# starkware-libs/stark-perpetual

Measured on AMD Instinct MI355X. Metric: pedersen_hashes_per_sec, higher is better.
Workload: dtype u32x9; 1 GPU; 2^16-leaf Pedersen Merkle rebuild per GPU (BASELINE.json configs[1]), 63 rebuilds in lockstep; tree_height=16, leaves_per_gpu=65536, calls_per_region=28, streams=2, window_bits=26, combine=none

## Files before the change

stark-perpetual_amd/csrc/pedersen.hip:

```cpp
#include <algorithm>
#include <cstdlib>
#include <cstring>
#include <map>
#include <vector>

#include "context.hpp"
#include "pedersen.hpp"
#include "quad.hpp"
#include "ragged_plan.hpp"

#ifndef SP_ACC_WAVES
#define SP_ACC_WAVES 1
#endif

namespace sp {

struct raw_aff {
  u256 x, y;
};
__device__ __forceinline__ raw_aff ld_raw(const aff_packed* e) {
  const uint4* q = reinterpret_cast<const uint4*>(e);
  const uint4 a = q[0], b = q[1], c = q[2], d = q[3];
  raw_aff r;
  r.x.w[0] = a.x; r.x.w[1] = a.y; r.x.w[2] = a.z; r.x.w[3] = a.w;
// ... 364 lines not shown
  const int wa = (upper && cnt >= 3) ? q + 2 * QUADS : q;
  const int wb = (upper && cnt >= 4) ? q + 3 * QUADS : q + QUADS;
  const aff pa = entry(wa), pb = entry(wb);
  qpt p = qmmadd(pa.x, pa.y, pb.x, pb.y, k);
  if (upper && cnt == 3) {
    p.a = odd ? pa.y : pa.x;
    p.b = FE_ONE_M;
  }
  qpt s = qadd<false>(p, k);
  if (cnt == 2) {
    s.a = fe_dpp<quad_perm(0, 1, 0, 1)>(p.a);
    s.b = fe_dpp<quad_perm(0, 1, 0, 1)>(p.b);
  }
  for (int j = 4; j < max_cnt; ++j) {
    const aff pj = entry(j < cnt ? q + j * QUADS : q);
    qpt t;
    t.a = fe_sel(upper, odd ? pj.y : pj.x, s.a);
    t.b = fe_sel(upper, FE_ONE_M, s.b);
    const qpt u = qadd<false>(t, k);
    if (j < cnt) s = u;
  }
#define SP_BUTTERFLY(XORV, LAST)                               \
  {                                                            \
    qpt t;                                                     \
    t.a = fe_sel(upper, fe_swizzle_xor<XORV>(s.a), s.a);       \
    t.b = fe_sel(upper, fe_swizzle_xor<XORV>(s.b), s.b);       \
    s = qadd<LAST>(t, k);                                      \
  }
  if constexpr (LOG_Q == 1) SP_BUTTERFLY(4, true)
  if constexpr (LOG_Q == 2) { SP_BUTTERFLY(4, false) SP_BUTTERFLY(8, true) }
  if constexpr (LOG_Q == 3) { SP_BUTTERFLY(4, false) SP_BUTTERFLY(8, false) SP_BUTTERFLY(16, true) }
#undef SP_BUTTERFLY
  const fe zinv = fe_inv_quad<true>(s.b, k);
  *unhashable = limbs_is_zero(zinv);
  return fe_pack(fe_canon(fe_mul(s.a, zinv)));
}

template <int LOG_Q, bool SPARSE = false>
__global__ void __launch_bounds__(256)
ped_quad_kernel(const uint64_t* __restrict__ x, const uint64_t* __restrict__ y, size_t xstride, size_t ystride,
                size_t n, const aff_packed* __restrict__ ped, int w0, int log2e, int nwin_plan,
                uint8_t* __restrict__ status, unsigned* __restrict__ flag, const int2* __restrict__ src,
                uint64_t* __restrict__ out, size_t ostride, int dup, const aff_packed* __restrict__ cpts, int cx,
                int cy) {
  constexpr int QUADS = 1 << LOG_Q, LANES = 4 * QUADS;
  const size_t gt = (size_t)blockIdx.x * blockDim.x + threadIdx.x;
  const size_t e_raw = gt / ((size_t)LANES << dup);
  const int g = (int)(gt % LANES);
  const bool active = e_raw < n;
  const size_t e = active ? e_raw : n - 1;
  const uint64_t *fx, *fy;
  operand_pointers(x, y, xstride, ystride, src, e, fx, fy);
  int mode = 0;
  if constexpr (SPARSE) {
    const int2 sc = src[e];
    mode = sc.x < 0 ? 1 : (sc.y < 0 ? 2 : 0);
  }
  bool unhashable;
  const u256 xa_plain = quad_hash<LOG_Q, SPARSE>(fx, fy, mode, cpts, cx, cy, ped, w0, log2e, nwin_plan, g, &unhashable);
  uint8_t st = unhashable ? SP_HASH_UNHASHABLE : SP_HASH_OK;
  if (!active || g != 0) return;
  if (!u256_lt(ld_u256(fx), U256_P) || !u256_lt(ld_u256(fy), U256_P)) st = SP_HASH_OUT_OF_RANGE;
  st_u256(out + 4 * e * ostride, xa_plain);
  if (status) status[e] = st;
  if (st != SP_HASH_OK && flag) atomicOr(flag, (unsigned)st);
}

template <int LOG_Q, bool SPARSE>
__global__ void __launch_bounds__(256)
ped_path_kernel(uint64_t* __restrict__ felts, const uint64_t* __restrict__ emp, size_t n,
                const aff_packed* __restrict__ ped, int w0, int log2e, int nwin_plan, unsigned* __restrict__ flag,
                const int2* __restrict__ src_all, PathLevels pl, int dup, const aff_packed* __restrict__ cpts_tree,
                int cx, int cy) {
  constexpr int QUADS = 1 << LOG_Q, LANES = 4 * QUADS;
  __shared__ uint64_t slot[256 / LANES][4];
  const size_t gt = (size_t)blockIdx.x * blockDim.x + threadIdx.x;
  const size_t e_raw = gt / ((size_t)LANES << dup);
  const int g = (int)(gt % LANES), grp = (int)(threadIdx.x / LANES);
  const bool active = e_raw < n;
  const size_t e = active ? e_raw : n - 1;
  for (int i = 0; i < pl.n_levels; ++i) {
    const int l = pl.first + i;
    const int2 sc = src_all[pl.src_off[l] + e];
    const uint64_t* y = emp + 4 * l;
    const uint64_t* fx = sc.x >= 0 ? felts + 4 * (size_t)sc.x : y;
    const uint64_t* fy = sc.y >= 0 ? felts + 4 * (size_t)sc.y : y;
    if (i > 0) {
      if (sc.x == pl.val_base[l] + (int)e) fx = slot[grp];
      else fy = slot[grp];
    }
    int mode = 0;
    if constexpr (SPARSE) mode = sc.x < 0 ? 1 : (sc.y < 0 ? 2 : 0);
    bool unhashable;
    const u256 xa = quad_hash<LOG_Q, SPARSE>(fx, fy, mode, cpts_tree ? cpts_tree + 2 * l : nullptr, cx, cy, ped, w0, log2e,
                                             nwin_plan, g, &unhashable);
    uint8_t st = unhashable ? SP_HASH_UNHASHABLE : SP_HASH_OK;
    if (i == 0 && g == 0 && (!u256_lt(ld_u256(fx), U256_P) || !u256_lt(ld_u256(fy), U256_P))) st = SP_HASH_OUT_OF_RANGE;
    __syncthreads();
    if (g == 0) {
      uint32_t* sl = reinterpret_cast<uint32_t*>(slot[grp]);
#pragma unroll
      for (int w = 0; w < 8; ++w) sl[w] = xa.w[w];
      if (active) {
        st_u256(felts + 4 * ((size_t)pl.val_base[l + 1] + e), xa);
        if (st != SP_HASH_OK && flag) atomicOr(flag, (unsigned)st);
      }
    }
    __syncthreads();
  }
}

template <int LOG_Q>
__global__ void __launch_bounds__(256)
ped_chain_kernel(const uint64_t* __restrict__ first, const uint64_t* __restrict__ words, long long word_stride, size_t n,
                 int steps, bool h_right, const aff_packed* __restrict__ ped, int w0, int log2e, int nwin_plan,
                 unsigned* __restrict__ flag, uint64_t* __restrict__ out, int dup) {
  constexpr int QUADS = 1 << LOG_Q, LANES = 4 * QUADS;
  __shared__ uint64_t slot[256 / LANES][4];
  const size_t gt = (size_t)blockIdx.x * blockDim.x + threadIdx.x;
  const size_t e_raw = gt / ((size_t)LANES << dup);
  const int g = (int)(gt % LANES), grp = (int)(threadIdx.x / LANES);
  const bool active = e_raw < n;
  const size_t e = active ? e_raw : n - 1;
  const uint64_t* h = first + 4 * e;
  const uint64_t* w = words + 4 * e;
  for (int j = 0; j < steps; ++j, w += 4 * word_stride) {
    const uint64_t* fx = h_right ? w : h;
    const uint64_t* fy = h_right ? h : w;
    bool unhashable;
    const u256 xa = quad_hash<LOG_Q, false>(fx, fy, 0, nullptr, 0, 0, ped, w0, log2e, nwin_plan, g, &unhashable);
    uint8_t st = unhashable ? SP_HASH_UNHASHABLE : SP_HASH_OK;
    if (g == 0 && (!u256_lt(ld_u256(w), U256_P) || (j == 0 && !u256_lt(ld_u256(h), U256_P)))) st = SP_HASH_OUT_OF_RANGE;
    __syncthreads();
    if (g == 0) {
      uint32_t* sl = reinterpret_cast<uint32_t*>(slot[grp]);
#pragma unroll
      for (int k = 0; k < 8; ++k) sl[k] = xa.w[k];
      if (active) {
        if (j == steps - 1) st_u256(out + 4 * e, xa);
        if (st != SP_HASH_OK && flag) atomicOr(flag, (unsigned)st);
      }
    }
    __syncthreads();
    h = slot[grp];
  }
}

__device__ __forceinline__ bool u256_same(const u256& a, const u256& b) {
  uint32_t d = 0;
#pragma unroll
  for (int k = 0; k < 8; ++k) d |= a.w[k] ^ b.w[k];
  return d == 0;
}
template <bool SIDED>
__device__ __forceinline__ void fold_result(size_t e, const u256& v, uint8_t st, uint64_t* __restrict__ out,
                                            uint8_t* __restrict__ status, const uint64_t* __restrict__ expect,
                                            size_t estride, uint8_t* __restrict__ verdict) {
  st_u256(out + 4 * e, v);
  if (status) status[e] = st;
  if constexpr (SIDED) {
    if (verdict) verdict[e] = (st == SP_HASH_OK && u256_same(v, ld_u256(expect + 4 * e * estride))) ? SP_PATH_TRUE : SP_PATH_FALSE;
  }
}

template <int LOG_Q, bool SIDED>
__global__ void __launch_bounds__(256)
ped_fold_ragged_kernel(const uint64_t* __restrict__ leaves, const uint64_t* __restrict__ words,
                       const uint32_t* __restrict__ off, const uint64_t* __restrict__ keys, size_t n,
                       const aff_packed* __restrict__ ped, int w0, int log2e, int nwin_plan, unsigned* __restrict__ flag,
                       uint8_t* __restrict__ status, uint64_t* __restrict__ out, const uint64_t* __restrict__ expect,
                       size_t estride, uint8_t* __restrict__ verdict, int dup) {
  constexpr int QUADS = 1 << LOG_Q, LANES = 4 * QUADS;
  __shared__ uint64_t slot[256 / LANES][4];
  __shared__ int block_steps;
  const size_t gt = (size_t)blockIdx.x * blockDim.x + threadIdx.x;
  const size_t e_raw = gt / ((size_t)LANES << dup);
  const int g = (int)(gt % LANES), grp = (int)(threadIdx.x / LANES);
  const bool active = e_raw < n;
  const size_t e = active ? e_raw : n - 1;
  const bool writer = active && g == 0 && ((gt / LANES) & (((size_t)1 << dup) - 1)) == 0;
  const uint32_t o0 = off[e];
  const int steps = (int)(off[e + 1] - o0) - (SIDED ? 0 : 1);
  uint64_t key = 0;
  if constexpr (SIDED) key = keys[e];
  if (threadIdx.x == 0) block_steps = 0;
  __syncthreads();
  if (g == 0 && steps > 0) atomicMax(&block_steps, steps);
  __syncthreads();
  const int bound = block_steps;
  const uint64_t* leaf = SIDED ? leaves + 4 * e : words + 4 * (size_t)o0;
  uint8_t st = SP_HASH_OK;
  if (steps == 0 && writer) {
    const u256 v = ld_u256(leaf);
    if (!u256_lt(v, U256_P)) st = SP_HASH_OUT_OF_RANGE;
    fold_result<SIDED>(e, v, st, out, status, expect, estride, verdict);
    if (st != SP_HASH_OK && flag) atomicOr(flag, (unsigned)st);
  }
  const uint64_t* h = leaf;
  const uint64_t* w = SIDED ? words + 4 * (size_t)o0 : leaf + 4;
  for (int j = 0; j < bound; ++j, w += 4) {
    const bool live = j < steps;
    const bool right = SIDED && ((key >> (j & 63)) & 1) != 0;
    const uint64_t* fx = live ? (right ? w : h) : leaf;
    const uint64_t* fy = live ? (right ? h : w) : leaf;
    bool unhashable;
    const u256 xa = quad_hash<LOG_Q, false>(fx, fy, 0, nullptr, 0, 0, ped, w0, log2e, nwin_plan, g, &unhashable);
    if (live && g == 0) {
      if (!u256_lt(ld_u256(w), U256_P) || (j == 0 && !u256_lt(ld_u256(h), U256_P))) st |= SP_HASH_OUT_OF_RANGE;
      else if (unhashable) st |= SP_HASH_UNHASHABLE;
    }
    __syncthreads();
    if (live && g == 0) {
      uint32_t* sl = reinterpret_cast<uint32_t*>(slot[grp]);
#pragma unroll
      for (int k = 0; k < 8; ++k) sl[k] = xa.w[k];
      if (j == steps - 1 && writer) {
        fold_result<SIDED>(e, xa, st, out, status, expect, estride, verdict);
        if (st != SP_HASH_OK && flag) atomicOr(flag, (unsigned)st);
      }
    }
    __syncthreads();
    h = slot[grp];
  }
}

__global__ void __launch_bounds__(256)
ped_fold_ragged_scatter_kernel(const uint64_t* __restrict__ work, const uint64_t* __restrict__ lone, bool sided,
                               const uint32_t* __restrict__ off, const uint32_t* __restrict__ perm,
                               const uint32_t* __restrict__ step_off, const uint8_t* __restrict__ step_status, size_t n,
                               unsigned* __restrict__ flag, uint8_t* __restrict__ status, uint64_t* __restrict__ out,
                               const uint64_t* __restrict__ expect, size_t estride, uint8_t* __restrict__ verdict) {
  const size_t k = (size_t)blockIdx.x * blockDim.x + threadIdx.x;
  if (k >= n) return;
  const uint32_t c = perm[k];
  const uint32_t o0 = off[c], steps = off[c + 1] - o0 - (sided ? 0 : 1);
  uint8_t st = SP_HASH_OK;
  u256 v;
  if (steps == 0) {
    v = ld_u256(lone + 4 * (size_t)(sided ? c : o0));
    if (!u256_lt(v, U256_P)) st = SP_HASH_OUT_OF_RANGE;
    if (st != SP_HASH_OK && flag) atomicOr(flag, (unsigned)st);
  } else {
    v = ld_u256(work + 4 * k);
    for (uint32_t s = 0; s < steps; ++s) st |= step_status[(size_t)step_off[s] + k];
  }
  fold_result<true>(c, v, st, out, status, expect, estride, verdict);
}

__global__ void __launch_bounds__(256)
ped_top_kernel(uint64_t* __restrict__ cur, size_t n_in, int n_levels, const aff_packed* __restrict__ ped, int w0, int log2e,
               int nwin_plan, unsigned* __restrict__ flag) {
  constexpr int LANES = 32, GROUPS = 256 / LANES;
  __shared__ uint64_t slot[2][GROUPS][4];
  const int g = (int)(threadIdx.x % LANES), grp = (int)(threadIdx.x / LANES);
  const size_t b = blockIdx.x;
  const int chunk = 1 << n_levels;
  uint64_t* out = cur + 4 * n_in;
  size_t n_out = n_in >> 1;
  int share = 4 - n_levels;
  for (int t = 0; t < n_levels; ++t, ++share) {
    const int cnt = chunk >> (t + 1);
    const int i = grp >> share;
    const bool writer = g == 0 && (grp & ((1 << share) - 1)) == 0;
    const uint64_t *fx, *fy;
    if (t == 0) {
      fx = cur + 4 * ((size_t)chunk * b + 2 * (size_t)i);
      fy = fx + 4;
    } else {
      fx = slot[(t - 1) & 1][2 * i];
      fy = slot[(t - 1) & 1][2 * i + 1];
    }
    bool unhashable;
    const u256 xa = quad_hash<3, false>(fx, fy, 0, nullptr, 0, 0, ped, w0, log2e, nwin_plan, g, &unhashable);
    uint8_t st = unhashable ? SP_HASH_UNHASHABLE : SP_HASH_OK;
    if (t == 0 && writer && (!u256_lt(ld_u256(fx), U256_P) || !u256_lt(ld_u256(fy), U256_P))) st = SP_HASH_OUT_OF_RANGE;
    if (writer) {
      uint32_t* sl = reinterpret_cast<uint32_t*>(slot[t & 1][i]);
#pragma unroll
      for (int w = 0; w < 8; ++w) sl[w] = xa.w[w];
      st_u256(out + 4 * ((size_t)cnt * b + (size_t)i), xa);
      if (st != SP_HASH_OK && flag) atomicOr(flag, (unsigned)st);
    }
    __syncthreads();
    out += 4 * n_out;
    n_out >>= 1;
  }
}

template <int S>
__device__ __forceinline__ u256 tail_hash(const uint64_t* fx, const uint64_t* fy, int lane, const aff_packed* __restrict__ ped,
                                          int w0, int log2e, int nwin, uint8_t* st) {
  if constexpr (S < 3) {
    return split_fused_x<S>(split_accumulate<S>(fx, fy, lane, ped, w0, log2e, nwin), st);
  } else {
    bool unhashable;
    const u256 xa = quad_hash<S - 2, false>(fx, fy, 0, nullptr, 0, 0, ped, w0, log2e, nwin, lane, &unhashable);
    if (unhashable) *st = SP_HASH_UNHASHABLE;
    return xa;
  }
}

__global__ void __launch_bounds__(256)
ped_tail_kernel(uint64_t* __restrict__ cur, size_t n_in, int s0, int n_levels, const aff_packed* __restrict__ ped, int w0,
                int log2e, int nwin_plan, unsigned* __restrict__ flag) {
  __shared__ uint64_t slot[2][256][4];
  const size_t b = blockIdx.x;
  const int tid = (int)threadIdx.x;
  uint64_t* out = cur + 4 * n_in;
  size_t n_out = n_in >> 1;
#pragma unroll 1
  for (int t = 0; t < n_levels; ++t) {
    const int s = s0 + t;
    const int cls = s < 5 ? s : 5;
    const int cnt = 256 >> s;
    const int i = tid >> s, lane = tid & ((1 << cls) - 1);
    const bool writer = (tid & ((1 << s) - 1)) == 0;
    const uint64_t *fx, *fy;
    if (t == 0) {
      fx = cur + 4 * (2 * (size_t)cnt * b + 2 * (size_t)i);
      fy = fx + 4;
    } else {
      fx = slot[(t - 1) & 1][2 * i];
      fy = slot[(t - 1) & 1][2 * i + 1];
    }
    uint8_t st = SP_HASH_OK;
    u256 xa;
    switch (cls) {
      case 0: xa = tail_hash<0>(fx, fy, lane, ped, w0, log2e, nwin_plan, &st); break;
      case 1: xa = tail_hash<1>(fx, fy, lane, ped, w0, log2e, nwin_plan, &st); break;
      case 2: xa = tail_hash<2>(fx, fy, lane, ped, w0, log2e, nwin_plan, &st); break;
      case 3: xa = tail_hash<3>(fx, fy, lane, ped, w0, log2e, nwin_plan, &st); break;
      case 4: xa = tail_hash<4>(fx, fy, lane, ped, w0, log2e, nwin_plan, &st); break;
      default: xa = tail_hash<5>(fx, fy, lane, ped, w0, log2e, nwin_plan, &st); break;
    }
    if (t == 0 && writer && (!u256_lt(ld_u256(fx), U256_P) || !u256_lt(ld_u256(fy), U256_P))) st = SP_HASH_OUT_OF_RANGE;
    if (writer) {
      uint32_t* sl = reinterpret_cast<uint32_t*>(slot[t & 1][i]);
#pragma unroll
      for (int w = 0; w < 8; ++w) sl[w] = xa.w[w];
      st_u256(out + 4 * ((size_t)cnt * b + (size_t)i), xa);
      if (st != SP_HASH_OK && flag) atomicOr(flag, (unsigned)st);
    }
    __syncthreads();
    out += 4 * n_out;
    n_out >>= 1;
  }
}

__global__ void __launch_bounds__(256)
ped_finish_kernel(const int32_t* __restrict__ sX, int32_t* __restrict__ sZZ, int32_t* __restrict__ sPre,
                  size_t n, size_t T, uint64_t* __restrict__ out, size_t ostride,
                  uint8_t* __restrict__ status, unsigned* __restrict__ flag) {
  const size_t t = (size_t)blockIdx.x * blockDim.x + threadIdx.x;
  if (t >= T) return;
  const size_t cnt = t < n ? (n - t + T - 1) / T : 0;
  fe run = FE_ONE_M;
  if (cnt > 0) {
    fe znext = load_limbs(sZZ, n, t);
#pragma unroll 1
    for (size_t j = 0; j < cnt; ++j) {
      const size_t e = t + j * T;
      const fe z = znext;
      if (j + 1 < cnt) znext = load_limbs(sZZ, n, e + T);
      store_limbs(sPre, n, e, run);
      run = fe_mul(run, z);
    }
  }
  if (fe_is_zero(run)) {
    run = FE_ONE_M;
#pragma unroll 1
    for (size_t e = t; e < n; e += T) {
      fe z = load_limbs(sZZ, n, e);
      if (fe_is_zero(z)) {
        z = FE_ONE_M;
        store_limbs(sZZ, n, e, z);
        if (status) status[e] = SP_HASH_UNHASHABLE;
        if (flag) atomicOr(flag, (unsigned)SP_HASH_UNHASHABLE);
      }
      store_limbs(sPre, n, e, run);
      run = fe_mul(run, z);
    }
  }
  size_t e = cnt > 0 ? t + (cnt - 1) * T : 0;
  fe zn = run, pn = run, xn = run;
  if (cnt > 0) {
    zn = load_limbs(sZZ, n, e);
    pn = load_limbs(sPre, n, e);
    xn = load_limbs(sX, n, e);
  }
  fe inv = fe_inv_shared_quad<2, true>(run, (int)(threadIdx.x & 3));
#pragma unroll 1
  for (size_t j = cnt; j-- > 0;) {
    const fe z = zn, pre = pn, xv = xn;
    const size_t cur = t + j * T;
    if (j > 0) {
      zn = load_limbs(sZZ, n, cur - T);
      pn = load_limbs(sPre, n, cur - T);
      xn = load_limbs(sX, n, cur - T);
    }
    const fe zinv = fe_mul(inv, pre);
    inv = fe_mul(inv, z);
    const fe xa = fe_mul(xv, zinv);
    st_u256(out + 4 * cur * ostride, fe_pack(fe_canon(xa)));
  }
}

template <bool Z_IN_LDS>
__global__ void __launch_bounds__(256)
ped_finish_lds_kernel(const int32_t* __restrict__ sX, int32_t* __restrict__ sZZ, size_t n, size_t T,
                      uint64_t* __restrict__ out, size_t ostride, uint8_t* __restrict__ status,
                      unsigned* __restrict__ flag, int kmax) {
  extern __shared__ int32_t fin_lds[];
  int32_t* lpre = fin_lds;
  int32_t* lz = fin_lds + (size_t)kmax * NL * 256;
  auto lds_put = [&](int32_t* base, size_t j, const fe& v) {
#pragma unroll
    for (int k = 0; k < NL; ++k) base[((j * NL + k) << 8) + threadIdx.x] = v.l[k];
  };
  auto lds_get = [&](const int32_t* base, size_t j) {
    fe v;
#pragma unroll
    for (int k = 0; k < NL; ++k) v.l[k] = base[((j * NL + k) << 8) + threadIdx.x];
    return v;
  };
  const size_t t = (size_t)blockIdx.x * blockDim.x + threadIdx.x;
  if (t >= T) return;
  const size_t cnt = t < n ? (n - t + T - 1) / T : 0;
  fe run = FE_ONE_M;
  if (cnt > 0) {
    fe znext = load_limbs(sZZ, n, t);
#pragma unroll 1
    for (size_t j = 0; j < cnt; ++j) {
      const fe z = znext;
      if (j + 1 < cnt) znext = load_limbs(sZZ, n, t + (j + 1) * T);
      lds_put(lpre, j, run);
      if (Z_IN_LDS) lds_put(lz, j, z);
      run = fe_mul(run, z);
    }
  }
  if (fe_is_zero(run)) {
    run = FE_ONE_M;
    size_t j = 0;
#pragma unroll 1
    for (size_t e = t; e < n; e += T, ++j) {
      fe z = load_limbs(sZZ, n, e);
      if (fe_is_zero(z)) {
        z = FE_ONE_M;
        store_limbs(sZZ, n, e, z);
        if (status) status[e] = SP_HASH_UNHASHABLE;
        if (flag) atomicOr(flag, (unsigned)SP_HASH_UNHASHABLE);
      }
      lds_put(lpre, j, run);
      if (Z_IN_LDS) lds_put(lz, j, z);
      run = fe_mul(run, z);
    }
  }
  size_t e = cnt > 0 ? t + (cnt - 1) * T : 0;
  fe zn = run, xn = run;
  if (cnt > 0) {
    if (!Z_IN_LDS) zn = load_limbs(sZZ, n, e);
    xn = load_limbs(sX, n, e);
  }
  fe inv = fe_inv_shared_quad<2, true>(run, (int)(threadIdx.x & 3));
#pragma unroll 1
  for (size_t j = cnt; j-- > 0;) {
    const fe z = Z_IN_LDS ? lds_get(lz, j) : zn, xv = xn;
    const fe pre = lds_get(lpre, j);
    const size_t cur = t + j * T;
    if (j > 0) {
      if (!Z_IN_LDS) zn = load_limbs(sZZ, n, cur - T);
      xn = load_limbs(sX, n, cur - T);
    }
    const fe zinv = fe_mul(inv, pre);
    inv = fe_mul(inv, z);
    const fe xa = fe_mul(xv, zinv);
    st_u256(out + 4 * cur * ostride, fe_pack(fe_canon(xa)));
  }
}

__global__ void __launch_bounds__(128)
ped_point_kernel(const uint64_t* __restrict__ x, const uint64_t* __restrict__ y, size_t n,
                 const aff_packed* __restrict__ ped, int w0, int log2e, int nwin,
                 uint64_t* __restrict__ ox, uint64_t* __restrict__ oy, uint8_t* __restrict__ status) {
  size_t e = (size_t)blockIdx.x * blockDim.x + threadIdx.x;
  if (e >= n) e = n - 1;
  u256 sx = ld_u256(x + 4 * e);
  u256 sy = ld_u256(y + 4 * e);
  if (!u256_lt(sx, U256_P) || !u256_lt(sy, U256_P)) {
    status[e] = SP_HASH_OUT_OF_RANGE;
    return;
  }
  bits512 str = concat_xy(sx, sy);
  xyzz acc = xyzz_from_aff(ld_aff(ped + pop_bits(str, w0)));
  for (int g = 1; g < nwin; ++g) {
    const window_ref r = window_entry(ped, g, pop_bits(str, log2e + 1), w0, log2e);
    acc = xyzz_madd(acc, signed_aff(ld_raw(r.entry), r.negative));
  }
  if (fe_is_zero(acc.ZZ)) {
    status[e] = SP_HASH_UNHASHABLE;
    return;
  }
  const fe izzz = fe_inv(acc.ZZZ);
  st_u256(ox + 4 * e, fe_pack(fe_from_mont(fe_mul(acc.X, fe_sqr(fe_mul(acc.ZZ, izzz))))));
  st_u256(oy + 4 * e, fe_pack(fe_from_mont(fe_mul(acc.Y, izzz))));
  status[e] = SP_HASH_OK;
}

__global__ void __launch_bounds__(64)
ped_partial_kernel(const uint64_t* __restrict__ felts, int count, const aff_packed* __restrict__ ped, int w0, int log2e,
                   int nwin, int cx, int cy, aff_packed* __restrict__ out) {
  int t = (int)(blockIdx.x * blockDim.x + threadIdx.x);
  if (t >= 2 * count) t = 2 * count - 1;
  const int side = t & 1;
  const uint64_t* f = felts + 4 * (size_t)(t >> 1);
  const int g0 = side == 0 ? 0 : nwin - cy, g1 = side == 0 ? cx : nwin;
  auto entry = [&](int w) {
    const window_ref r =
        window_entry(ped, w, window_from_memory(f, f, window_start(w, w0, log2e), window_width(w, w0, log2e)), w0, log2e);
    return signed_aff(ld_raw(r.entry), r.negative);
  };
  aff_packed res;
  if (g1 - g0 == 1) {
    const aff a = entry(g0);
    res.x = fe_pack(fe_canon(a.x));
    res.y = fe_pack(fe_canon(a.y));
  } else {
    xyzz acc = xyzz_mmadd(entry(g0), entry(g0 + 1));
    for (int g = g0 + 2; g < g1; ++g) acc = xyzz_madd(acc, entry(g));
    const fe izzz = fe_inv(acc.ZZZ);
    const fe izz = fe_sqr(fe_mul(acc.ZZ, izzz));
    res.x = fe_pack(fe_canon(fe_mul(acc.X, izz)));
    res.y = fe_pack(fe_canon(fe_mul(acc.Y, izzz)));
  }
  uint4* q = reinterpret_cast<uint4*>(out + t);
  q[0] = make_uint4(res.x.w[0], res.x.w[1], res.x.w[2], res.x.w[3]);
  q[1] = make_uint4(res.x.w[4], res.x.w[5], res.x.w[6], res.x.w[7]);
  q[2] = make_uint4(res.y.w[0], res.y.w[1], res.y.w[2], res.y.w[3]);
  q[3] = make_uint4(res.y.w[4], res.y.w[5], res.y.w[6], res.y.w[7]);
}

struct KernelProfile {
  bool enabled = false;
  std::vector<hipEvent_t> ev;
  std::vector<size_t> units;
  size_t used = 0;
};
static KernelProfile g_prof;
bool profile_launch_begin(hipStream_t st) {
  if (!g_prof.enabled || g_prof.used + 2 > g_prof.ev.size()) return false;
  (void)hipEventRecord(g_prof.ev[g_prof.used], st);
  return true;
}
void profile_launch_end(hipStream_t st, size_t units) {
  (void)hipEventRecord(g_prof.ev[g_prof.used + 1], st);
  g_prof.units.push_back(units);
  g_prof.used += 2;
}
static bool g_split_enabled = getenv("STARKPERP_NO_SPLIT") == nullptr;
static bool g_fuse_enabled = getenv("STARKPERP_NO_FUSE") == nullptr;
static bool g_quad_enabled = getenv("STARKPERP_NO_QUAD") == nullptr;
static bool g_quad2_enabled = getenv("STARKPERP_NO_QUAD2") == nullptr;
static bool g_level_split = getenv("STARKPERP_NO_LEVEL_SPLIT") == nullptr;
static bool g_quad_no_dup = getenv("STARKPERP_QUAD_NO_DUP") != nullptr;
static bool g_sparse_enabled = getenv("STARKPERP_NO_SPARSE_LEVELS") == nullptr;
static size_t g_quad_max = getenv("STARKPERP_QUAD_MAX") ? (size_t)atoll(getenv("STARKPERP_QUAD_MAX")) : 2048;
static size_t quad_class_max(int log_q, int nwin) {
  if (!g_quad_enabled || nwin > 64) return 0;
  if (log_q == 3) return nwin >= 16 ? g_quad_max : 0;
  if (log_q == 2) return nwin >= 8 ? 2 * g_quad_max : 0;
  return nwin >= 4 && g_quad2_enabled ? 4 * g_quad_max : 0;
}
struct QuadShape {
  int log_q, dup;
  unsigned blocks;
};
static QuadShape quad_shape(size_t n, int nwin) {
  QuadShape q{0, 0, 0};
  for (int l = 3; l >= 1 && q.log_q == 0; --l) {
    if (n <= quad_class_max(l, nwin)) q.log_q = l;
  }
  if (q.log_q == 0) return q;
  while ((4 << (q.log_q + q.dup)) < 64 && ((n * 4) << (q.log_q + q.dup + 1)) <= 65536) ++q.dup;
  if (g_quad_no_dup) q.dup = 0;
  q.blocks = (unsigned)((((n * 4) << (q.log_q + q.dup)) + 255) / 256);
  return q;
}
template <class F>
static void dispatch_quad(int log_q, bool sparse, F&& launch) {
  using std::integral_constant;
  if (sparse && log_q == 2) launch(integral_constant<int, 2>{}, std::true_type{});
  else if (sparse) launch(integral_constant<int, 1>{}, std::true_type{});
  else if (log_q == 3) launch(integral_constant<int, 3>{}, std::false_type{});
  else if (log_q == 2) launch(integral_constant<int, 2>{}, std::false_type{});
  else launch(integral_constant<int, 1>{}, std::false_type{});
}

static std::map<StreamKey, DeviceBuffer> g_stream_scratch;
static int get_scratch(size_t n, Scratch& s, hipStream_t st) { return get_scratch_public(n, s, st); }
static int get_scratch_tail(size_t n, size_t tail_bytes, Scratch& s, char** tail, hipStream_t st) {
  DeviceBuffer& buf = g_stream_scratch[stream_key(st)];
  const size_t plane = ((9 * n * sizeof(int32_t)) + 255) & ~(size_t)255;
  SP_HIP(buf.reserve(3 * plane + 256 + tail_bytes));
  char* b = (char*)buf.ptr;
  s.X = (int32_t*)b;
  s.ZZ = (int32_t*)(b + plane);
  s.Pre = (int32_t*)(b + 2 * plane);
  s.flag = (unsigned*)(b + 3 * plane);
  if (tail) *tail = b + 3 * plane + 256;
  return SP_OK;
}
int get_scratch_public(size_t n, Scratch& s, hipStream_t st) { return get_scratch_tail(n, 0, s, nullptr, st); }

static size_t g_finish_lanes = getenv("STARKPERP_FINISH_LANES") ? (size_t)atoll(getenv("STARKPERP_FINISH_LANES")) : 65536;
static size_t parse_split_lanes() {
  const char* e = getenv("STARKPERP_SPLIT_LANES");
  long long v = e ? atoll(e) : 65536;
  if (v < 256) v = 256;
  if (v > (1ll << 24)) v = 1ll << 24;
  return ((size_t)v + 255) & ~(size_t)255;
}
static size_t g_split_lanes = parse_split_lanes();
static bool g_finish_lds = getenv("STARKPERP_NO_FINISH_LDS") == nullptr;
static int finish_lds_ready() {
  static std::map<int, int> done;
  int dev = -1;
  if (hipGetDevice(&dev) != hipSuccess) return SP_ERR_HIP;
  auto it = done.find(dev);
  if (it != done.end()) return it->second;
  const int want = 16 * NL * 256 * (int)sizeof(int32_t);
  hipError_t e = hipFuncSetAttribute(reinterpret_cast<const void*>(ped_finish_lds_kernel<true>),
                                     hipFuncAttributeMaxDynamicSharedMemorySize, want);
  if (e == hipSuccess)
    e = hipFuncSetAttribute(reinterpret_cast<const void*>(ped_finish_lds_kernel<false>),
                            hipFuncAttributeMaxDynamicSharedMemorySize, want);
  if (e != hipSuccess) (void)hipGetLastError();
  return done[dev] = (e == hipSuccess ? SP_OK : SP_ERR_HIP);
}
static size_t finish_threads(size_t n) {
  size_t K = (n + g_finish_lanes - 1) / g_finish_lanes;
  if (K < 1) K = 1;
  if (K > 32) K = 32;
  return ((n + K - 1) / K + 3) & ~(size_t)3;
}

void release_ragged_stage();
void release_pedersen_state() {
  for (auto& kv : g_stream_scratch) kv.second.release();
  g_stream_scratch.clear();
  release_ragged_stage();
  for (hipEvent_t e : g_prof.ev) (void)hipEventDestroy(e);
  g_prof.ev.clear();
  g_prof.units.clear();
  g_prof.used = 0;
  g_prof.enabled = false;
}

void constant_window_counts(const PedPlan& p, int& cx, int& cy) {
  cx = cy = 0;
  for (int g = 0; g < p.nwin; ++g) {
    if (p.start[g] + p.bits[g] <= 252) ++cx;
    if (p.start[g] >= 252) ++cy;
  }
}
static bool sparse_class(const PedPlan& plan, int log_q, int& cx, int& cy) {
  if (!g_sparse_enabled || (log_q != 1 && log_q != 2)) return false;
  constant_window_counts(plan, cx, cy);
  const int shortest = 1 + plan.nwin - (cx > cy ? cx : cy);
  return cx >= 1 && cy >= 1 && shortest >= (2 << log_q);
}
int enqueue_partial_points(const uint64_t* felts, int count, aff_packed* out, hipStream_t st, bool* usable) {
  Context& c = ctx();
  int cx, cy;
  constant_window_counts(c.plan, cx, cy);
  *usable = cx >= 1 && cy >= 1 && count > 0;
  if (!*usable) return SP_OK;
  hipLaunchKernelGGL(ped_partial_kernel, dim3((unsigned)((2 * count + 63) / 64)), dim3(64), 0, st, felts, count, c.ped,
                     (int)c.plan.bits[0], c.plan.log2e, c.plan.nwin, cx, cy, out);
  SP_HIP(hipGetLastError());
  return SP_OK;
}

static int split_log_l(size_t n, int nwin) {
  int log_l = 0;
  if (g_split_enabled) {
    if (n * 8 <= g_split_lanes) log_l = 3;
    else if (n * 4 <= g_split_lanes) log_l = 2;
    else if (n * 2 <= g_split_lanes) log_l = 1;
    while (log_l > 0 && nwin < (2 << log_l)) --log_l;
  }
  return log_l;
}
static int tail_lane_class(size_t n, int nwin) {
  const QuadShape q = quad_shape(n, nwin);
  if (q.log_q != 0) return 2 + q.log_q;
  const int log_l = split_log_l(n, nwin);
  const bool one_launch = g_split_enabled && g_fuse_enabled && log_l <= 2 && (n << log_l) <= 65536;
  return one_launch ? log_l : -1;
}

static int enqueue_pedersen_impl(const uint64_t* x, size_t xs, const uint64_t* y, size_t ys, uint64_t* out,
                                 size_t os, uint8_t* status, unsigned* flag, size_t n, hipStream_t st,
                                 const Scratch& s, const int2* src, const aff_packed* cpts);
int enqueue_pedersen(const uint64_t* x, size_t xs, const uint64_t* y, size_t ys, uint64_t* out,
                     size_t os, uint8_t* status, unsigned* flag, size_t n, hipStream_t st,
                     const Scratch& s, const int2* src) {
  return enqueue_pedersen_impl(x, xs, y, ys, out, os, status, flag, n, st, s, src, nullptr);
}
int enqueue_pedersen_sparse(const uint64_t* x, const uint64_t* y, uint64_t* out, unsigned* flag, size_t n,
                            hipStream_t st, const Scratch& s, const int2* src, const aff_packed* cpts) {
  return enqueue_pedersen_impl(x, 1, y, 1, out, 1, nullptr, flag, n, st, s, src, cpts);
}
static bool g_path_fusion = getenv("STARKPERP_NO_PATH_FUSION") == nullptr;
static bool g_top_fusion = getenv("STARKPERP_NO_TOP_FUSION") == nullptr;
static bool g_tail_fusion = getenv("STARKPERP_NO_TAIL_FUSION") == nullptr;
static bool g_chain_fusion = getenv("STARKPERP_NO_CHAIN_FUSION") == nullptr;
int enqueue_pedersen_chain(const uint64_t* first, const uint64_t* words, long long word_stride, size_t n, size_t steps,
                           bool h_right, uint64_t* out, unsigned* flag, hipStream_t st, bool* done) {
  *done = false;
  Context& c = ctx();
  const int w0 = c.plan.bits[0], log2e = c.plan.log2e, nwin = c.plan.nwin;
  if (!g_chain_fusion || n == 0 || steps < 2 || steps > 0x7fffffffull) return SP_OK;
  const QuadShape q = quad_shape(n, nwin);
  if (q.log_q == 0) return SP_OK;
  dispatch_quad(q.log_q, false, [&](auto Q, auto) {
    hipLaunchKernelGGL((ped_chain_kernel<decltype(Q)::value>), dim3(q.blocks), dim3(256), 0, st, first, words, word_stride,
                       n, (int)steps, h_right, c.ped, w0, log2e, nwin, flag, out, q.dup);
  });
  SP_HIP(hipGetLastError());
  *done = true;
  return SP_OK;
}
int enqueue_pedersen_top(uint64_t* cur, size_t n_in, unsigned remaining, unsigned* flag, hipStream_t st, int* levels_done) {
  *levels_done = 0;
  Context& c = ctx();
  const int nwin = c.plan.nwin;
  if (g_tail_fusion && nwin >= 16 && nwin <= 64 && n_in >= 2) {
    const int s0 = tail_lane_class(n_in / 2, nwin);
    const int L = 9 - s0;
    bool take = s0 >= 0 && s0 <= 4 && remaining >= (unsigned)L;
    for (int t = 1; take && t < L; ++t) take = tail_lane_class(n_in >> (t + 1), nwin) == (s0 + t < 5 ? s0 + t : 5);
    if (take) {
      hipLaunchKernelGGL(ped_tail_kernel, dim3((unsigned)(n_in >> L)), dim3(256), 0, st, cur, n_in, s0, L, c.ped,
                         (int)c.plan.bits[0], c.plan.log2e, nwin, flag);
      SP_HIP(hipGetLastError());
      *levels_done = L;
      return SP_OK;
    }
  }
  if (!g_top_fusion || !g_quad_enabled || nwin > 64 || nwin < 16 || remaining < 2 || n_in / 2 > g_quad_max || n_in < 4) return SP_OK;
  const int L = remaining < 4 ? (int)remaining : 4;
  const unsigned blocks = (unsigned)(n_in >> L);
  hipLaunchKernelGGL(ped_top_kernel, dim3(blocks), dim3(256), 0, st, cur, n_in, L, c.ped, (int)c.plan.bits[0], c.plan.log2e,
                     nwin, flag);
  SP_HIP(hipGetLastError());
  *levels_done = L;
  return SP_OK;
}
int enqueue_pedersen_path(uint64_t* felts, const uint64_t* emp, unsigned* flag, size_t n, hipStream_t st,
                          const int2* src_all, const PathLevels& pl, const aff_packed* cpts_tree, bool* done) {
  *done = false;
  Context& c = ctx();
  const int w0 = c.plan.bits[0], log2e = c.plan.log2e, nwin = c.plan.nwin;
  if (!g_path_fusion || n == 0 || pl.n_levels < 2) return SP_OK;
  const QuadShape q = quad_shape(n, nwin);
  if (q.log_q == 0) return SP_OK;
  int cx = 0, cy = 0;
  const bool sparse = cpts_tree != nullptr && sparse_class(c.plan, q.log_q, cx, cy);
  dispatch_quad(q.log_q, sparse, [&](auto Q, auto S) {
    hipLaunchKernelGGL((ped_path_kernel<decltype(Q)::value, decltype(S)::value>), dim3(q.blocks), dim3(256), 0, st, felts,
                       emp, n, c.ped, w0, log2e, nwin, flag, src_all, pl, q.dup, sparse ? cpts_tree : nullptr, cx, cy);
  });
  SP_HIP(hipGetLastError());
  *done = true;
  return SP_OK;
}

static int enqueue_pedersen_impl(const uint64_t* x, size_t xs, const uint64_t* y, size_t ys, uint64_t* out,
                                 size_t os, uint8_t* status, unsigned* flag, size_t n, hipStream_t st,
                                 const Scratch& s, const int2* src, const aff_packed* cpts) {
  if (n == 0) return SP_OK;
  Context& c = ctx();
  bool prof = false;
  const int w0 = c.plan.bits[0], log2e = c.plan.log2e, nwin = c.plan.nwin;
  const int log_l = split_log_l(n, nwin);
  bool fused = false;
  const QuadShape q = quad_shape(n, nwin);
  if (q.log_q != 0) {
    int cx = 0, cy = 0;
    const bool sparse = cpts != nullptr && src != nullptr && sparse_class(c.plan, q.log_q, cx, cy);
    dispatch_quad(q.log_q, sparse, [&](auto Q, auto S) {
      hipLaunchKernelGGL((ped_quad_kernel<decltype(Q)::value, decltype(S)::value>), dim3(q.blocks), dim3(256), 0, st, x, y,
                         xs, ys, n, c.ped, w0, log2e, nwin, status, flag, src, out, os, q.dup, cpts, cx, cy);
    });
    fused = true;
  } else if (log_l == 0 && !(g_split_enabled && g_fuse_enabled && n <= 65536)) {
    size_t n_bulk = n, rem = 0;
    int rem_l = 0;
    if (g_level_split && g_split_enabled && n > g_split_lanes && (n % g_split_lanes) != 0 &&
        (n % g_split_lanes) * 2 <= g_split_lanes) {
      rem = n % g_split_lanes;
      rem_l = rem * 8 <= g_split_lanes ? 3 : (rem * 4 <= g_split_lanes ? 2 : 1);
      while (rem_l > 0 && nwin < (2 << rem_l)) --rem_l;
      if (rem_l == 0) rem = 0;
      n_bulk = n - rem;
    }
    if (rem == 0) {
      prof = g_prof.enabled && g_prof.used + 2 <= g_prof.ev.size() && n > 65536;
      if (prof) (void)hipEventRecord(g_prof.ev[g_prof.used], st);
      hipLaunchKernelGGL(ped_accumulate_kernel, dim3((unsigned)((n_bulk + 255) / 256)), dim3(256), 0, st, x, y, xs, ys,
                         n_bulk, c.ped, w0, log2e, nwin, s.X, s.ZZ, status, flag, src, n);
    } else {
      const unsigned bulk_blocks = (unsigned)(n_bulk / 256);
      const unsigned rblocks = (unsigned)(((rem << rem_l) + 255) / 256);
#define SP_LAUNCH_MIXED(LOGL)                                                                                     \
  hipLaunchKernelGGL((ped_accumulate_mixed_kernel<LOGL>), dim3(bulk_blocks + rblocks), dim3(256), 0, st, x, y, xs, \
                     ys, n_bulk, rem, bulk_blocks, c.ped, w0, log2e, nwin, s.X, s.ZZ, status, flag, src, n)
      if (rem_l == 3) SP_LAUNCH_MIXED(3);
      else if (rem_l == 2) SP_LAUNCH_MIXED(2);
      else SP_LAUNCH_MIXED(1);
#undef SP_LAUNCH_MIXED
    }
    if (prof) {
      (void)hipEventRecord(g_prof.ev[g_prof.used + 1], st);
      g_prof.units.push_back(n);
      g_prof.used += 2;
    }
  } else {
    const unsigned blocks = (unsigned)(((n << log_l) + 255) / 256);
    fused = g_fuse_enabled && (n << log_l) <= 65536;
#define SP_LAUNCH_SPLIT(LOGL, FUSEDV)                                                                      \
  hipLaunchKernelGGL((ped_accumulate_split_kernel<LOGL, FUSEDV>), dim3(blocks), dim3(256), 0, st, x, y, xs, \
                     ys, n, c.ped, w0, log2e, nwin, s.X, s.ZZ, status, flag, src, out, os, n)
    if (log_l == 0) SP_LAUNCH_SPLIT(0, true);
    else if (log_l == 3) { if (fused) SP_LAUNCH_SPLIT(3, true); else SP_LAUNCH_SPLIT(3, false); }
    else if (log_l == 2) { if (fused) SP_LAUNCH_SPLIT(2, true); else SP_LAUNCH_SPLIT(2, false); }
    else { if (fused) SP_LAUNCH_SPLIT(1, true); else SP_LAUNCH_SPLIT(1, false); }
#undef SP_LAUNCH_SPLIT
  }
  if (!fused) {
    const size_t T = finish_threads(n);
    const unsigned tpb = T >= 256 ? 256 : 64;
    const unsigned blocksB = (unsigned)((T + tpb - 1) / tpb);
    const size_t kmax = (n + T - 1) / T;
    if (g_finish_lds && tpb == 256 && kmax >= 2 && kmax <= 16 && finish_lds_ready() == SP_OK) {
      const bool z_too = kmax <= 8;
      const size_t lds_bytes = kmax * NL * 256 * sizeof(int32_t) * (z_too ? 2 : 1);
      if (z_too) hipLaunchKernelGGL((ped_finish_lds_kernel<true>), dim3(blocksB), dim3(256), lds_bytes, st, s.X, s.ZZ, n, T,
                                    out, os, status, flag, (int)kmax);
      else hipLaunchKernelGGL((ped_finish_lds_kernel<false>), dim3(blocksB), dim3(256), lds_bytes, st, s.X, s.ZZ, n, T,
                              out, os, status, flag, (int)kmax);
    } else {
      hipLaunchKernelGGL(ped_finish_kernel, dim3(blocksB), dim3(tpb), 0, st, s.X, s.ZZ, s.Pre, n, T, out,
                         os, status, flag);
    }
  }
  SP_HIP(hipGetLastError());
  return SP_OK;
}

static bool g_chain_ragged = getenv("STARKPERP_NO_CHAIN_RAGGED") == nullptr;
static bool g_path_fold = getenv("STARKPERP_NO_PATH_FOLD") == nullptr;
struct RaggedStage {
  PinnedBuffer host;
  hipEvent_t copied = nullptr;
  bool pending = false;
};
static std::map<StreamKey, RaggedStage> g_ragged_stage;
void release_ragged_stage() {
  for (auto& kv : g_ragged_stage) {
    if (kv.second.copied) (void)hipEventDestroy(kv.second.copied);
    kv.second.host.release();
  }
  g_ragged_stage.clear();
}
int stage_copy(std::initializer_list<Piece> pieces, void* dev, hipStream_t st) {
  RaggedStage& rs = g_ragged_stage[stream_key(st)];
  if (rs.pending) {
    SP_HIP(hipEventSynchronize(rs.copied));
    rs.pending = false;
  }
  if (rs.copied == nullptr) SP_HIP(hipEventCreateWithFlags(&rs.copied, hipEventDisableTiming));
  size_t bytes = 0;
  for (const Piece& p : pieces) bytes += p.bytes;
  SP_HIP(rs.host.reserve(bytes));
  size_t at = 0;
  for (const Piece& p : pieces) {
    if (p.bytes) std::memcpy((char*)rs.host.ptr + at, p.ptr, p.bytes);
    at += p.bytes;
  }
  SP_HIP(hipMemcpyAsync(dev, rs.host.ptr, bytes, hipMemcpyHostToDevice, st));
  SP_HIP(hipEventRecord(rs.copied, st));
  rs.pending = true;
  return SP_OK;
}
static size_t chain_ragged_cap() {
  if (!g_chain_ragged) return 0;
  const int nwin = ctx().plan.nwin;
  return std::max({quad_class_max(1, nwin), quad_class_max(2, nwin), quad_class_max(3, nwin)});
}
int enqueue_pedersen_fold_ragged(const uint64_t* leaves, const uint64_t* words, const uint32_t* off, const uint64_t* keys,
                                 size_t n, uint64_t* out, uint8_t* status, const uint64_t* expect, size_t estride,
                                 uint8_t* verdict, hipStream_t st) {
  if (n == 0) return SP_OK;
  Context& c = ctx();
  const int w0 = c.plan.bits[0], log2e = c.plan.log2e, nwin = c.plan.nwin;
  const bool sided = keys != nullptr;
  const size_t total = off[n];
  const size_t cap = sided && !g_path_fold ? 0 : chain_ragged_cap();
  Scratch s;
  char* tail = nullptr;
  if (cap != 0) {
    const size_t key_bytes = sided ? n * sizeof(uint64_t) : 0, off_bytes = (n + 1) * sizeof(uint32_t);
    int rc = get_scratch_tail(1, key_bytes + off_bytes, s, &tail, st);
    if (rc != SP_OK) return rc;
    SP_HIP(hipMemsetAsync(s.flag, 0, sizeof(unsigned), st));
    const uint64_t* d_keys = (const uint64_t*)tail;
    const uint32_t* d_off = (const uint32_t*)(tail + key_bytes);
    rc = stage_copy({{keys, key_bytes}, {off, off_bytes}}, tail, st);
    if (rc != SP_OK) return rc;
    for (size_t b = 0; b < n; b += cap) {
      const size_t m = n - b < cap ? n - b : cap;
      const QuadShape q = quad_shape(m, nwin);
      dispatch_quad(q.log_q, false, [&](auto Q, auto) {
        if (sided)
          hipLaunchKernelGGL((ped_fold_ragged_kernel<decltype(Q)::value, true>), dim3(q.blocks), dim3(256), 0, st,
                             leaves + 4 * b, words, d_off + b, d_keys + b, m, c.ped, w0, log2e, nwin, s.flag,
                             status ? status + b : nullptr, out + 4 * b, expect ? expect + 4 * b * estride : nullptr,
                             estride, verdict ? verdict + b : nullptr, q.dup);
        else
          hipLaunchKernelGGL((ped_fold_ragged_kernel<decltype(Q)::value, false>), dim3(q.blocks), dim3(256), 0, st,
                             nullptr, words, d_off + b, nullptr, m, c.ped, w0, log2e, nwin, s.flag,
                             status ? status + b : nullptr, out + 4 * b, nullptr, 0, nullptr, q.dup);
      });
      SP_HIP(hipGetLastError());
    }
    return SP_OK;
  }
  if (ragged_work_felts(off, n, sided) > 0x7fffffffull) {
    set_error(sided ? "merkle paths: more than 2^31 felts" : "ragged chains: more than 2^31 felts");
    return SP_ERR_BAD_ARGUMENT;
  }
  const RaggedPlan p = ragged_plan(off, keys, n);
  const size_t meta_bytes = (p.meta.size() * sizeof(uint32_t) + 255) & ~(size_t)255;
  const size_t stat_bytes = (p.n_pairs + 255) & ~(size_t)255;
  int rc = get_scratch_tail(n, meta_bytes + stat_bytes + p.work_felts * 32, s, &tail, st);
  if (rc != SP_OK) return rc;
  SP_HIP(hipMemsetAsync(s.flag, 0, sizeof(unsigned), st));
  uint32_t* d_meta = (uint32_t*)tail;
  uint8_t* d_stat = (uint8_t*)(tail + meta_bytes);
  uint64_t* d_work = (uint64_t*)(tail + meta_bytes + stat_bytes);
  rc = stage_copy({{p.meta.data(), p.meta.size() * sizeof(uint32_t)}}, d_meta, st);
  if (rc != SP_OK) return rc;
  if (sided) SP_HIP(hipMemcpyAsync(d_work + 4 * n, leaves, n * 32, hipMemcpyDeviceToDevice, st));
  if (total > 0) SP_HIP(hipMemcpyAsync(d_work + 4 * (p.work_felts - total), words, total * 32, hipMemcpyDeviceToDevice, st));
  const int2* d_pairs = reinterpret_cast<const int2*>(d_meta + p.pairs_at);
  for (size_t j = 0; j < p.max_steps; ++j) {
    rc = enqueue_pedersen(d_work, 1, d_work, 1, d_work, 1, d_stat + p.step_off()[j], s.flag, p.running[j], st, s,
                          d_pairs + p.step_off()[j]);
    if (rc != SP_OK) return rc;
  }
  hipLaunchKernelGGL(ped_fold_ragged_scatter_kernel, dim3((unsigned)((n + 255) / 256)), dim3(256), 0, st, d_work,
                     sided ? leaves : words, sided, d_meta, d_meta + n + 1, d_meta + 2 * n + 1, d_stat, n, s.flag, status, out,
                     expect, estride, verdict);
  SP_HIP(hipGetLastError());
  return SP_OK;
}
static bool ragged_offsets_ok(const uint32_t* off, size_t n) {
  if (off == nullptr || off[0] != 0) { set_error("ragged chains: off[0] must be 0"); return false; }
  for (size_t i = 0; i < n; ++i) {
    if (off[i + 1] <= off[i]) { set_error("ragged chains: every chain needs at least one element"); return false; }
  }
  return true;
}

static const uint32_t* path_offsets_ok(const uint32_t* off, unsigned height, const uint64_t* keys, size_t n,
                                       std::vector<uint32_t>& uniform) {
  if (keys == nullptr) { set_error("merkle paths: keys must not be NULL"); return nullptr; }
  if (off == nullptr) {
    if (height > 64) { set_error("merkle paths: height must be <= 64"); return nullptr; }
    if (height != 0 && n > 0xffffffffull / height) { set_error("merkle paths: more than 2^32 - 1 sibling felts"); return nullptr; }
    uniform.resize(n + 1);
    for (size_t i = 0; i <= n; ++i) uniform[i] = (uint32_t)(i * height);
    off = uniform.data();
  } else {
    if (off[0] != 0) { set_error("merkle paths: off[0] must be 0"); return nullptr; }
    for (size_t i = 0; i < n; ++i) {
      if (off[i + 1] < off[i]) { set_error("merkle paths: the offsets must not decrease"); return nullptr; }
      if (off[i + 1] - off[i] > 64) { set_error("merkle paths: a path has at most 64 siblings"); return nullptr; }
    }
  }
  for (size_t i = 0; i < n; ++i) {
    const uint32_t len = off[i + 1] - off[i];
    if (len < 64 && (keys[i] >> len) != 0) { set_error("merkle paths: a key bit at or above its path's length is set"); return nullptr; }
  }
  return off;
}
static int merkle_paths_host(const uint64_t* leaves, const uint64_t* siblings, const uint32_t* off, unsigned height,
                             const uint64_t* keys, size_t n, const uint64_t* expected, size_t n_expected, uint64_t* roots,
                             uint8_t* verdict, uint8_t* status) {
  LaneScope ls(0);
  SP_REQUIRE_READY();
  const bool verify = verdict != nullptr;
  if (verify && n_expected != 1 && n_expected != n) { set_error("merkle paths: n_expected must be 1 or n"); return SP_ERR_BAD_ARGUMENT; }
  if (n == 0) return SP_OK;
  std::vector<uint32_t> uniform;
  off = path_offsets_ok(off, height, keys, n, uniform);
  if (off == nullptr) return SP_ERR_BAD_ARGUMENT;
  if (ls.open() != SP_OK) return SP_ERR_HIP;
  HostLane& L = *ls.lane;
  const size_t total = off[n];
  const size_t n_exp = verify ? n_expected : 0;
  const size_t in_bytes = (n + total + n_exp) * 32;
  SP_HIP(L.io.reserve(in_bytes + n * 32 + 2 * n + 64));
  uint64_t* d_leaves = (uint64_t*)L.io.ptr;
  uint64_t* d_sib = d_leaves + 4 * n;
  uint64_t* d_exp = d_sib + 4 * total;
  uint64_t* d_roots = d_exp + 4 * n_exp;
  uint8_t* d_ver = (uint8_t*)(d_roots + 4 * n);
  uint8_t* d_st = d_ver + n;
  SP_HIP(hipMemcpyAsync(d_leaves, leaves, n * 32, hipMemcpyHostToDevice, L.stream));
  if (total > 0) SP_HIP(hipMemcpyAsync(d_sib, siblings, total * 32, hipMemcpyHostToDevice, L.stream));
  if (verify) SP_HIP(hipMemcpyAsync(d_exp, expected, n_exp * 32, hipMemcpyHostToDevice, L.stream));
  int rc;
  {
    ctx_lock lk(ctx().mu);
    rc = enqueue_pedersen_fold_ragged(d_leaves, d_sib, off, keys, n, d_roots, d_st, verify ? d_exp : nullptr,
                                      n_expected == n ? 1 : 0, verify ? d_ver : nullptr, L.stream);
  }
  if (rc != SP_OK) return rc;
  if (verify) {
    SP_HIP(hipMemcpyAsync(verdict, d_ver, n, hipMemcpyDeviceToHost, L.stream));
    if (status) SP_HIP(hipMemcpyAsync(status, d_st, n, hipMemcpyDeviceToHost, L.stream));
  } else {
    SP_HIP(hipMemcpyAsync(roots, d_roots, n * 32, hipMemcpyDeviceToHost, L.stream));
    if (status) SP_HIP(hipMemcpyAsync(status, d_st, n, hipMemcpyDeviceToHost, L.stream));
  }
  SP_HIP(hipStreamSynchronize(L.stream));
  return SP_OK;
}

}

using namespace sp;

extern "C" {

int sp_pedersen_batch_dev(const uint64_t* x, const uint64_t* y, uint64_t* out, uint8_t* status,
                          size_t n, void* stream) {
// ... 360 lines not shown
```

Measured before the change: 1.038 billion hashes/s.

## Fuse remaining top tree levels into tail kernel via last-block-climbs counters

After the tail kernel finishes its fused levels, each block increments an atomic counter for its group, and the last block to arrive in a group goes on to hash the next levels up the tree. This replaces the separate kernel launches that previously handled the top levels with a single launch. It adds per-stream counter buffers and release/acquire fences, and the topmost levels run on only a few blocks, so they are serialized behind the last arriving block.

```diff
diff --git a/stark-perpetual_amd/csrc/pedersen.hip b/stark-perpetual_amd/csrc/pedersen.hip
--- a/stark-perpetual_amd/csrc/pedersen.hip
+++ b/stark-perpetual_amd/csrc/pedersen.hip
@@ -690,14 +690,45 @@
 
 __global__ void __launch_bounds__(256)
 ped_tail_kernel(uint64_t* __restrict__ cur, size_t n_in, int s0, int n_levels, const aff_packed* __restrict__ ped, int w0,
-                int log2e, int nwin_plan, unsigned* __restrict__ flag) {
+                int log2e, int nwin_plan, unsigned* __restrict__ flag, unsigned* __restrict__ climb, int climb_left,
+                int climb_cap) {
   __shared__ uint64_t slot[2][256][4];
-  const size_t b = blockIdx.x;
+  __shared__ unsigned climb_last;
+  size_t b = blockIdx.x;
   const int tid = (int)threadIdx.x;
   uint64_t* out = cur + 4 * n_in;
   size_t n_out = n_in >> 1;
+  bool leaves = true;
 #pragma unroll 1
-  for (int t = 0; t < n_levels; ++t) {
+  for (int t = 0;; ++t) {
+    if (t == n_levels) {
+      if (climb_left == 0) break;
+      const int lg = climb_left < climb_cap ? climb_left : climb_cap;
+      const size_t grp = b >> lg;
+      if (tid == 0) {
+        asm volatile("s_waitcnt vmcnt(0)" ::: "memory");
+        __builtin_amdgcn_fence(__ATOMIC_RELEASE, "agent");
+        asm volatile("s_waitcnt vmcnt(0)" ::: "memory");
+        const unsigned ticket = __hip_atomic_fetch_add(climb + grp, 1u, __ATOMIC_RELAXED, __HIP_MEMORY_SCOPE_AGENT);
+        const bool last = ticket == (1u << lg) - 1;
+        if (last) {
+          __builtin_amdgcn_fence(__ATOMIC_ACQUIRE, "agent");
+          asm volatile("s_waitcnt vmcnt(0)" ::: "memory");
+          __hip_atomic_store(climb + grp, 0u, __ATOMIC_RELAXED, __HIP_MEMORY_SCOPE_AGENT);
+        }
+        climb_last = last ? 1u : 0u;
+      }
+      __syncthreads();
+      if (climb_last == 0) break;
+      climb += (2 * n_out) >> lg;
+      cur = out - 8 * n_out;
+      b = grp;
+      s0 = 9 - lg;
+      n_levels = lg;
+      climb_left -= lg;
+      leaves = false;
+      t = 0;
+    }
     const int s = s0 + t;
     const int cls = s < 5 ? s : 5;
     const int cnt = 256 >> s;
@@ -721,7 +752,8 @@
       case 4: xa = tail_hash<4>(fx, fy, lane, ped, w0, log2e, nwin_plan, &st); break;
       default: xa = tail_hash<5>(fx, fy, lane, ped, w0, log2e, nwin_plan, &st); break;
     }
-    if (t == 0 && writer && (!u256_lt(ld_u256(fx), U256_P) || !u256_lt(ld_u256(fy), U256_P))) st = SP_HASH_OUT_OF_RANGE;
+    if (leaves && t == 0 && writer && (!u256_lt(ld_u256(fx), U256_P) || !u256_lt(ld_u256(fy), U256_P)))
+      st = SP_HASH_OUT_OF_RANGE;
     if (writer) {
       uint32_t* sl = reinterpret_cast<uint32_t*>(slot[t & 1][i]);
 #pragma unroll
@@ -998,6 +1030,21 @@
   return SP_OK;
 }
 int get_scratch_public(size_t n, Scratch& s, hipStream_t st) { return get_scratch_tail(n, 0, s, nullptr, st); }
+constexpr size_t CLIMB_COUNTERS = 4096;
+static std::map<StreamKey, DeviceBuffer> g_climb_counters;
+static int get_climb_counters(unsigned** counters, hipStream_t st) {
+  DeviceBuffer& buf = g_climb_counters[stream_key(st)];
+  if (!buf.ptr) {
+    SP_HIP(buf.reserve(CLIMB_COUNTERS * sizeof(unsigned)));
+    const hipError_t e = hipMemsetAsync(buf.ptr, 0, buf.bytes, st);
+    if (e != hipSuccess) {
+      buf.release();
+      return hip_fail(e, "hipMemsetAsync(climb counters)");
+    }
+  }
+  *counters = (unsigned*)buf.ptr;
+  return SP_OK;
+}
 
 static size_t g_finish_lanes = getenv("STARKPERP_FINISH_LANES") ? (size_t)atoll(getenv("STARKPERP_FINISH_LANES")) : 65536;
 static size_t parse_split_lanes() {
@@ -1035,6 +1082,8 @@
 void release_pedersen_state() {
   for (auto& kv : g_stream_scratch) kv.second.release();
   g_stream_scratch.clear();
+  for (auto& kv : g_climb_counters) kv.second.release();
+  g_climb_counters.clear();
   release_ragged_stage();
   for (hipEvent_t e : g_prof.ev) (void)hipEventDestroy(e);
   g_prof.ev.clear();
@@ -1102,6 +1151,14 @@
 static bool g_top_fusion = getenv("STARKPERP_NO_TOP_FUSION") == nullptr;
 static bool g_tail_fusion = getenv("STARKPERP_NO_TAIL_FUSION") == nullptr;
 static bool g_chain_fusion = getenv("STARKPERP_NO_CHAIN_FUSION") == nullptr;
+static bool g_tail_climb = getenv("STARKPERP_NO_TAIL_CLIMB") == nullptr;
+static bool g_tail_climb_forests = getenv("STARKPERP_TAIL_CLIMB_FORESTS") != nullptr;
+static int parse_tail_climb_cap() {
+  const char* e = getenv("STARKPERP_TAIL_CLIMB_GROUP");
+  const int v = e ? atoi(e) : 4;
+  return v < 1 ? 1 : v > 9 ? 9 : v;
+}
+static int g_tail_climb_cap = parse_tail_climb_cap();
 int enqueue_pedersen_chain(const uint64_t* first, const uint64_t* words, long long word_stride, size_t n, size_t steps,
                            bool h_right, uint64_t* out, unsigned* flag, hipStream_t st, bool* done) {
   *done = false;
@@ -1128,10 +1185,26 @@
     bool take = s0 >= 0 && s0 <= 4 && remaining >= (unsigned)L;
     for (int t = 1; take && t < L; ++t) take = tail_lane_class(n_in >> (t + 1), nwin) == (s0 + t < 5 ? s0 + t : 5);
     if (take) {
-      hipLaunchKernelGGL(ped_tail_kernel, dim3((unsigned)(n_in >> L)), dim3(256), 0, st, cur, n_in, s0, L, c.ped,
-                         (int)c.plan.bits[0], c.plan.log2e, nwin, flag);
+      const size_t blocks = n_in >> L;
+      const bool lone = (n_in >> remaining) == 1;
+      int climb_left = g_tail_climb && (lone || g_tail_climb_forests) ? (int)remaining - L : 0;
+      size_t counters = 0;
+      for (int left = climb_left, sh = 0; left > 0;) {
+        const int lg = left < g_tail_climb_cap ? left : g_tail_climb_cap;
+        sh += lg;
+        left -= lg;
+        counters += blocks >> sh;
+      }
+      unsigned* climb = nullptr;
+      if (counters > CLIMB_COUNTERS) climb_left = 0;
+      if (climb_left > 0) {
+        const int rc = get_climb_counters(&climb, st);
+        if (rc != SP_OK) return rc;
+      }
+      hipLaunchKernelGGL(ped_tail_kernel, dim3((unsigned)blocks), dim3(256), 0, st, cur, n_in, s0, L, c.ped,
+                         (int)c.plan.bits[0], c.plan.log2e, nwin, flag, climb, climb_left, g_tail_climb_cap);
       SP_HIP(hipGetLastError());
-      *levels_done = L;
+      *levels_done = L + climb_left;
       return SP_OK;
     }
   }
```

After: 1.037 billion hashes/s. About the same (-0.1%).
